# olvb/phaze

Hardware: AMD Instinct MI355X
Metric: stft_frames_per_sec_1024pt_hop256_48k (higher is better)
Workload: dtype f32+f64; 1 GPU; C2: BASELINE configs[1], mono 48 kHz 1024/256 pf 1.5, 1 ch x 2^20 hops resident; fft=1024, hop=256, channels=1, frames_per_chunk=342, parallelism=streams x1, no collective, device=AMD Radeon Graphics (gfx950:sramecc+:xna

## Files before the change

include/phaze_amd.h:

```cpp
#ifndef PHAZE_AMD_H
#define PHAZE_AMD_H

#include <stddef.h>
#include <stdint.h>

#ifdef __cplusplus
extern "C" {
#endif

#if defined(__GNUC__)
#define PV_API __attribute__((visibility("default")))
#else
#define PV_API
#endif

enum {
    PV_OK = 0,
    PV_ERR_FFT_SIZE = 1,
    PV_ERR_ARGUMENT = 2,
    PV_ERR_UNSUPPORTED = 3,
    PV_ERR_CAPACITY = 4,
    PV_ERR_DEVICE = 5,
    PV_ERR_DESTROYED = 6
};
// ... 34 lines not shown
    int32_t compute_units, device_id;
    char device_name[64];
    char kernel_name[32];
} pv_info;

PV_API int pv_create(const pv_config *cfg, pv_handle **out);
PV_API int pv_abi_version(void);
PV_API int pv_destroy(pv_handle *h);

PV_API const char *pv_last_error(const pv_handle *h);
PV_API const char *pv_status_string(int status);
PV_API int pv_get_info(const pv_handle *h, pv_info *out);
PV_API int pv_device_count(int32_t *out);

PV_API int pv_forward_stats(pv_handle *h, uint64_t *frames, uint64_t *fallbacks, int32_t reset);

PV_API int pv_reset(pv_handle *h);
PV_API int pv_reset_channels(pv_handle *h, int32_t first, int32_t count);
enum { PV_STATE_HISTORY = 1, PV_STATE_ACCUMULATOR = 2 };
PV_API int pv_reset_channels_part(pv_handle *h, int32_t first, int32_t count, int32_t parts);
PV_API int pv_get_time_cursor(const pv_handle *h, int64_t *out);
PV_API int pv_set_time_cursor(pv_handle *h, int64_t value);

PV_API int pv_export_state(pv_handle *h, int32_t ch, float *hist, float *acc, int64_t *time_cursor);
PV_API int pv_import_state(pv_handle *h, int32_t ch, const float *hist, const float *acc, int64_t time_cursor);

PV_API int pv_process(pv_handle *h, const float *const *in, float *const *out, int32_t nch,
                      int32_t nsamples, float pitch_factor);

PV_API int pv_process_begin(pv_handle *h, const float *const *in, int32_t nch, int32_t nsamples, float pitch_factor);
// ... 133 lines not shown
```

phaze_amd/capi.py:

```python
import ctypes as C
import os
import subprocess
import sys

import numpy as np

_HERE = os.path.dirname(os.path.abspath(__file__))
_LIB_PATH = os.environ.get("PHAZE_LIB") or os.path.join(_HERE, "lib", "libphaze_amd.so")
_lib = None

PV_OK, PV_ERR_FFT_SIZE, PV_ERR_ARGUMENT, PV_ERR_UNSUPPORTED, PV_ERR_CAPACITY, PV_ERR_DEVICE, PV_ERR_DESTROYED = range(7)

EXPORTS = [
    "pv_create", "pv_destroy", "pv_last_error", "pv_status_string", "pv_get_info", "pv_reset", "pv_reset_channels",
    "pv_get_time_cursor", "pv_set_time_cursor", "pv_process", "pv_process_batch", "pv_process_batch_device",
    "pv_set_stream", "pv_synchronize", "pv_debug_frame", "pv_export_state", "pv_import_state", "pv_abi_version",
    "pv_process_begin", "pv_process_end", "pv_device_count", "pv_host_alloc", "pv_host_free", "pv_reset_channels_part",
    "pv_forward_stats",
    "pv_stretch_create", "pv_stretch_destroy", "pv_stretch_reset", "pv_stretch_last_error", "pv_stretch_process", "pv_stretch_process_device",
    "pv_stretch_set_stream", "pv_stretch_synchronize", "pv_stretch_export_state", "pv_stretch_import_state",
    "pv_tempo_process", "pv_tempo_process_device",
    "pv_link_channels",
    "pv_transient_process", "pv_transient_process_device", "pv_onset_strength", "pv_onset_strength_device", "pv_transient_plan",
    "pv_onsets_from_strength", "pv_transient_chain_layout", "pv_onset_chain_layout",
    "pv_resample_create", "pv_resample_destroy", "pv_resample_reset", "pv_resample_last_error", "pv_resample_set_stream", "pv_resample_synchronize",
    "pv_resample_process", "pv_resample_process_device", "pv_resample_out_count", "pv_resample_export_state", "pv_resample_import_state",
    "pv_resample_design", "pv_resample_count",
    "pv_pitch_create", "pv_pitch_destroy", "pv_pitch_reset", "pv_pitch_last_error", "pv_pitch_set_stream", "pv_pitch_synchronize",
    "pv_pitch_process", "pv_pitch_process_device", "pv_pitch_stretch", "pv_pitch_resampler",
]


class PvError(RuntimeError):
# ... 150 lines not shown
    L.pv_pitch_stretch.argtypes = [vp]
    L.pv_pitch_resampler.argtypes = [vp]
    for n in EXPORTS:
        if n not in ("pv_last_error", "pv_status_string", "pv_stretch_last_error"):
            getattr(L, n).restype = C.c_int
    L.pv_onsets_from_strength.restype = L.pv_transient_plan.restype = C.c_int64
    L.pv_resample_design.restype = L.pv_resample_count.restype = C.c_int64
    L.pv_resample_last_error.restype = L.pv_pitch_last_error.restype = C.c_char_p
    L.pv_pitch_stretch.restype = L.pv_pitch_resampler.restype = vp
    L.pv_process_begin.argtypes = [vp, C.POINTER(fp), C.c_int32, C.c_int32, C.c_float]
    L.pv_process_end.argtypes = [vp, C.POINTER(fp)]
    L.pv_device_count.argtypes = [C.POINTER(C.c_int32)]
    L.pv_host_alloc.argtypes = [C.c_size_t, C.POINTER(vp)]
    L.pv_host_free.argtypes = [vp]
    L.pv_forward_stats.argtypes = [vp, C.POINTER(C.c_uint64), C.POINTER(C.c_uint64), C.c_int32]
    L.pv_abi_version.argtypes = []
    if L.pv_abi_version() != ABI_VERSION:
        raise PvError(PV_ERR_ARGUMENT, f"{_LIB_PATH} has PV_ABI_VERSION {L.pv_abi_version()}, this binding expects {ABI_VERSION}: rebuild the library")
    _lib = L
    return L


def _fp(a):
    return a.ctypes.data_as(C.POINTER(C.c_float))


class _PinnedBlock:

    def __init__(self, nbytes):
        self._L = load_library()
# ... 198 lines not shown
    def process_batch_device(self, d_in, d_out, nch, nhops, ch_stride, d_pitch, pitch_stride=0, channels_per_stream=1):
        self._check(self._L.pv_process_batch_device(self._h, C.c_void_p(d_in), C.c_void_p(d_out), nch, nhops, ch_stride,
                                                    C.c_void_p(d_pitch), pitch_stride, channels_per_stream))

    def set_stream(self, hip_stream):
        self._check(self._L.pv_set_stream(self._h, C.c_void_p(hip_stream)))

    def synchronize(self):
        self._check(self._L.pv_synchronize(self._h))

    def forward_stats(self, reset=False):
        a, b = C.c_uint64(0), C.c_uint64(0)
        self._check(self._L.pv_forward_stats(self._h, C.byref(a), C.byref(b), 1 if reset else 0))
        return int(a.value), int(b.value)

    def debug_frame(self, ch, block, pitch):
        N = self.fft_size
        H = N // 2 + 1
        block = np.ascontiguousarray(block, dtype=np.float32)
        X = np.zeros(2 * N, dtype=np.float64)
        mag = np.zeros(H, dtype=np.float32)
        flags = np.zeros(H, dtype=np.int32)
        Y = np.zeros(2 * H, dtype=np.float32)
        self._check(self._L.pv_debug_frame(self._h, ch, _fp(block), C.c_float(float(pitch)), X.ctypes.data_as(C.POINTER(C.c_double)),
                                           _fp(mag), flags.ctypes.data_as(C.POINTER(C.c_int32)), _fp(Y)))
        return {"X": X, "mag": mag, "flags": flags, "Y": Y}


def tempo_hops(tempo, synthesis_hop, min_hop, max_hop, carry=0.0):
    t = np.atleast_1d(np.asarray(tempo, np.float64))
# ... 467 lines not shown
```

phaze_amd/csrc/pv_capi.hip:

```cpp
#include <hip/hip_runtime.h>
#include <math.h>
#include <stdio.h>
#include <stdlib.h>
#include <string.h>

#include <atomic>
#include <chrono>
#include <vector>
#if defined(__x86_64__)
#include <immintrin.h>
#endif

#include "../../include/phaze_amd.h"
#include "pv_kernels.h"

namespace {
constexpr uint32_t kMagic = 0x50564d49u;
constexpr int kHdrFloats = 16;
constexpr int kMaxPieces = 16;
constexpr int kFwdStatWords = 1024;
thread_local char g_create_err[256] = "";
}

struct pv_handle {
    uint32_t magic;
    int N, hop, L, R, log2n;
    int max_channels, max_hops, device, cus;
    int frames_per_chunk_cfg;
    int last_frames_per_chunk;
    hipStream_t own_stream, stream;
    double2 *d_tw64;
    float2 *d_tw32;
    float *d_hann;
    float *d_hist[2], *d_acc[2];
    int cur;
    float *d_stage_in, *d_stage_out, *d_pitch;
    unsigned *d_chain_list;
    long chain_list_cap;
    int chain_list_flip = 0;
    unsigned char *d_gscratch;
    size_t gscratch_cap;
    float *d_snap;
    size_t snap_floats;
    unsigned idle_ticks;
// ... 52 lines not shown
int fail_hip(pv_handle *h, hipError_t e, const char *what)
{
    char buf[256];
    snprintf(buf, sizeof buf, "%s: %s", what, hipGetErrorString(e));
    return fail(h, PV_ERR_DEVICE, buf);
}

#define HIPCHK(h, call)                                            \
    do {                                                           \
        hipError_t e_ = (call);                                    \
        if (e_ != hipSuccess) return fail_hip((h), e_, #call);     \
    } while (0)

bool live(const pv_handle *h) { return h && h->magic == kMagic; }

int pick_frames_per_chunk(const pv_handle *h, int nch, int nhops)
{
    if (h->frames_per_chunk_cfg > 0) return h->frames_per_chunk_cfg;
    long per_cu;
    if (h->use_wave2k) per_cu = pv_wave2k_threads() / 64;
    else if (h->use_wave) per_cu = pv_wave_threads() / 64;
    else if (h->use_wg) { per_cu = (160 * 1024) / (long)(pv_wg_lds_bytes(h->log2n, h->hop, !h->use_wg16) + 256); if (per_cu < 1) per_cu = 1; }
    else { per_cu = (160 * 1024) / (long)pv_kernel_lds_bytes(h->log2n, h->hop); if (per_cu > 8) per_cu = 8; if (per_cu < 1) per_cu = 1; }
    const long resident = per_cu * h->cus;
    const int R = h->R;
    int best = R > 1 ? R : 1;
    double best_eff = -1.0;
    auto consider = [&](int F) {
        if (F < 1) return;
        const long chunks = (nhops + F - 1) / F;
        const long chains = (long)nch * chunks;
        const long rounds = (chains + resident - 1) / resident;
        const double fill = (double)chains / (double)(rounds * resident);
        const double halo = (double)nhops / (double)(nhops + (chunks - 1) * (R - 1));
        const double eff = fill * halo;
        if (eff > best_eff + 1e-9) { best_eff = eff; best = F; }
// ... 6 lines not shown
    for (int F = 48 * R; F >= (R > 1 ? R : 1); F -= (F > 8 * R ? R : 1)) {
        if (F > nhops && F > R) continue;
        consider(F);
    }
    if (best > nhops) best = nhops;
    return best < 1 ? 1 : best;
}

int launch_chain(pv_handle *h, const float *d_in, float *d_out, int ch0, int nch, int nhops, long ch_stride, const float *d_pitch,
                 int pitch_stride, int ch_per_stream, bool chunked, int dbg_ch, unsigned done_seq, int spread = -1)
{
    PvKernelParams p;
    memset(&p, 0, sizeof p);
    p.in = d_in; p.out = d_out; p.ch_stride = ch_stride;
    p.nhops = nhops; p.hop = h->hop;
    p.frames_per_chunk = chunked ? pick_frames_per_chunk(h, nch, nhops) : nhops;
    p.pitch = d_pitch; p.pitch_stride = pitch_stride; p.ch_per_stream = ch_per_stream > 0 ? ch_per_stream : 1;
    const size_t soff = (size_t)ch0 * h->L;
    p.hist_in = h->d_hist[h->cur] + soff; p.hist_out = h->d_hist[h->cur ^ 1] + soff;
    p.acc_in = h->d_acc[h->cur] + soff;   p.acc_out = h->d_acc[h->cur ^ 1] + soff;
    p.t0_mod_n = (int)(h->time_cursor & (int64_t)(h->N - 1));
    p.tw64 = h->d_tw64; p.tw32 = h->d_tw32; p.hann = h->d_hann;
    p.dbg_ch = -1; p.dbg_frame = -1;
    p.fwd64 = h->fwd64 ? 1 : 0; p.fwd_stats = h->d_fwd_stats;
    if (done_seq) { p.done = h->d_done; p.done_seq = done_seq; }
#ifdef PV_STAMPS
    p.stamps = h->d_stamps;
#endif
    if (dbg_ch >= 0) { p.dbg_X = h->d_dbgX; p.dbg_mag = h->d_dbgMag; p.dbg_flags = h->d_dbgFlags; p.dbg_Y = h->d_dbgY; p.dbg_ch = dbg_ch; p.dbg_frame = 0; }
    const int nchunks = (nhops + p.frames_per_chunk - 1) / p.frames_per_chunk;
    h->last_frames_per_chunk = p.frames_per_chunk;
// ... 22 lines not shown
        if (!h->use_wave && !h->use_wg) {
            const size_t stride = pv_kernel_gscratch_bytes(h->log2n, h->hop);
            if (stride) {
                const size_t need = stride * (size_t)nch * (size_t)nchunks;
                if (need > ((size_t)16 << 30)) return fail(h, PV_ERR_CAPACITY, "fft_size >= 16384: the launch needs more than 16 GiB of scratch (fewer channels or hops per call)");
                if (need > h->gscratch_cap) {
                    HIPCHK(h, hipStreamSynchronize(h->stream));
                    if (h->d_gscratch) (void)hipFree(h->d_gscratch);
                    h->d_gscratch = nullptr; h->gscratch_cap = 0;
                    HIPCHK(h, hipMalloc(&h->d_gscratch, need));
                    h->gscratch_cap = need;
                }
                p.gscratch = h->d_gscratch; p.gscratch_stride = stride;
            }
        }
        e = h->use_wave ? pv_launch_wave(p, nch, nchunks, h->stream, spread, list, list_next)
          : h->use_wg ? pv_launch_wg(h->log2n, p, nch, nchunks, h->stream, !h->use_wg16)
                      : pv_launch_chain(h->log2n, p, nch, nchunks, h->stream);
    }
    if (e != hipSuccess) return fail_hip(h, e, "kernel launch");
    return PV_OK;
}

int commit_chain(pv_handle *h, int nch, int nhops)
{
    if (nch > h->used_channels) h->used_channels = nch;
    if (nch < h->used_channels && h->L > 0) {
        const size_t off = (size_t)nch * h->L, cnt = (size_t)(h->used_channels - nch) * h->L * sizeof(float);
        HIPCHK(h, hipMemcpyAsync(h->d_hist[h->cur ^ 1] + off, h->d_hist[h->cur] + off, cnt, hipMemcpyDeviceToDevice, h->stream));
        HIPCHK(h, hipMemcpyAsync(h->d_acc[h->cur ^ 1] + off, h->d_acc[h->cur] + off, cnt, hipMemcpyDeviceToDevice, h->stream));
    }
    h->cur ^= 1;
    h->time_cursor += (int64_t)nhops * h->hop;
// ... 445 lines not shown
int pv_forward_stats(pv_handle *h, uint64_t *frames, uint64_t *fallbacks, int32_t reset)
{
    if (!live(h)) return PV_ERR_DESTROYED;
    { const int rs_ = resident_stop(h); if (rs_ != PV_OK) return rs_; }
    HIPCHK(h, hipSetDevice(h->device));
    HIPCHK(h, hipStreamSynchronize(h->stream));
    unsigned long long st[256];
    HIPCHK(h, hipMemcpy(st, h->d_fwd_stats, sizeof st, hipMemcpyDeviceToHost));
    uint64_t a = 0, b = 0;
    for (int i = 0; i < 128; i++) { a += st[2 * i]; b += st[2 * i + 1]; }
    if (frames) *frames = a;
    if (fallbacks) *fallbacks = b;
    if (reset) HIPCHK(h, hipMemset(h->d_fwd_stats, 0, sizeof(unsigned long long) * kFwdStatWords));
    return PV_OK;
}

#ifdef PV_FLIP_COUNT
PV_API int pv_exp_flip_stats(pv_handle *h, uint64_t *out)
{
    if (!live(h) || !out) return PV_ERR_ARGUMENT;
    HIPCHK(h, hipSetDevice(h->device));
    HIPCHK(h, hipStreamSynchronize(h->stream));
    unsigned long long st[kFwdStatWords];
    HIPCHK(h, hipMemcpy(st, h->d_fwd_stats, sizeof st, hipMemcpyDeviceToHost));
    for (int k = 0; k < 12; k++) out[k] = 0;
    for (int i = 0; i < 128; i++) { out[0] += st[2 * i]; out[1] += st[2 * i + 1]; out[2] += st[256 + 2 * i]; out[3] += st[257 + 2 * i]; }
    for (int k = 0; k < 6; k++) out[4 + k] = st[512 + k] & 0xFFFFFFFFull;
    out[10] = st[600]; out[11] = st[601];
    return PV_OK;
}
// ... 333 lines not shown
```

phaze_amd/csrc/pv_kernels.h:

```cpp
#pragma once
#include <hip/hip_runtime.h>
#include <stddef.h>
#include <atomic>

struct PvKernelParams {
    const float *in;
    float *out;
    long ch_stride;
    int nhops;
    int hop;
    int frames_per_chunk;
    int nchunks;
    int nch;
    const float *pitch;
    int pitch_stride;
    int ch_per_stream;
    const float *hist_in;
    float *hist_out;
    const float *acc_in;
    float *acc_out;
    int t0_mod_n;
    const double2 *tw64;
    const float2 *tw32;
    const float *hann;
// ... 40 lines not shown
inline PvKernelParams pv_resident_params(const PvKernelParams &p, int nslots)
{
    PvKernelParams q = p;
    q.nchunks = 1; q.nch = nslots; q.nhops = 1; q.frames_per_chunk = 1;
    return q;
}

int pv_kernel_threads(int log2n);
size_t pv_kernel_lds_bytes(int log2n, int hop);
size_t pv_kernel_gscratch_bytes(int log2n, int hop);
hipError_t pv_launch_chain(int log2n, const PvKernelParams &p, int nch, int nchunks, hipStream_t st);

size_t pv_wave_lds_bytes();
int pv_wave_threads();
bool pv_wave_supported(int log2n, int hop);
hipError_t pv_launch_wave(const PvKernelParams &p, int nch, int nchunks, hipStream_t st, int spread, unsigned *list, unsigned *list_next = nullptr);
hipError_t pv_launch_wave_resident(const PvKernelParams &p, int nslots, hipStream_t st);
hipError_t pv_launch_wave2k_resident(const PvKernelParams &p, int nslots, hipStream_t st);
bool pv_wg_resident_supported(int log2n, int hop, bool wg8);
hipError_t pv_launch_wg_resident(int log2n, const PvKernelParams &p, int nslots, hipStream_t st, bool wg8);

bool pv_wave2k_supported(int log2n, int hop);
size_t pv_wave2k_lds_bytes();
int pv_wave2k_threads();
hipError_t pv_launch_wave2k(const PvKernelParams &p, int nch, int nchunks, hipStream_t st);

bool pv_wg_supported(int log2n, int hop);
size_t pv_wg_lds_bytes(int log2n, int hop, bool wg8);
int pv_wg_threads(int log2n, int hop, bool wg8);
hipError_t pv_launch_wg(int log2n, const PvKernelParams &p, int nch, int nchunks, hipStream_t st, bool wg8);

bool pv_wg16_supported(int log2n, int hop);
// ... 6 lines not shown
```

phaze_amd/csrc/pv_wave_kernel.hip:

```cpp
#include <hip/hip_runtime.h>
#include <stdint.h>
#include <type_traits>

#include "pv_kernels.h"
#include "pv_device_common.h"
#include "pv_pk_math.h"
#include "pv_residue.h"
#include "pv_wave_fft.h"
#include "pv_guard.h"

namespace {

#ifndef PV_FP64_FLAVOUR
#define PV_FP64_FLAVOUR 0
#endif
#ifndef PV_WAVES
#define PV_WAVES (PV_FP64_FLAVOUR ? 8 : 12)
#endif
#ifndef PV_WAVES_PER_SIMD
#define PV_WAVES_PER_SIMD (PV_FP64_FLAVOUR ? 2 : 3)
#endif
constexpr bool FP64 = PV_FP64_FLAVOUR != 0;
constexpr int WAVES = PV_WAVES;
constexpr int RES_WAVES = 4;
// ... 1245 lines not shown
    __syncthreads();
    if (threadIdx.x == 0) {
        unsigned n[2] = {0u, 0u};
        for (int w = 0; w < CLS_WAVES; w++) if (cls_of[w] < 2u) n[cls_of[w]]++;
        base[0] = n[0] ? atomicAdd(&list[0], n[0]) : 0u;
        base[1] = n[1] ? atomicAdd(&list[1], n[1]) : 0u;
    }
    __syncthreads();
    if (l == 0 && cls < 2u) {
        unsigned before = 0;
        for (int w = 0; w < wv; w++) before += (cls_of[w] == cls) ? 1u : 0u;
        list[2 + cls * nchains + base[cls] + before] = (unsigned)chain;
    }
}

template <int S_ROWS, bool AUX>
hipError_t launch_wave(const PvKernelParams &p, int nch, int nchunks, hipStream_t st, int spread, unsigned *list, unsigned *list_next)
{
    constexpr bool F32OK = !AUX && !FP64;
    const bool f32 = F32OK && !p.fwd64;
    PvKernelParams q = p;
    q.nchunks = nchunks;
    q.nch = nch;
    const long chains = (long)nch * nchunks;
    const dim3 grid((unsigned)((chains + WAVES - 1) / WAVES), 1, 1), block(64 * WAVES, 1, 1);
    const size_t lds = pv_wave_lds_bytes();
    auto k = [&] { return f32 ? pv_launch_instance<pv_wave_kernel_1024<S_ROWS, AUX, false, false, F32OK>>(grid, block, lds, st, q)
                              : pv_launch_instance<pv_wave_kernel_1024<S_ROWS, AUX, false, false, false>>(grid, block, lds, st, q); };
    auto ks = [&] { return f32 ? pv_launch_instance<pv_wave_kernel_1024<S_ROWS, false, false, true, F32OK>>(grid, block, lds, st, q)
                               : pv_launch_instance<pv_wave_kernel_1024<S_ROWS, false, false, true>>(grid, block, lds, st, q); };
    if (FP64 && !AUX) return ks();
    if (AUX || spread == 0 || (spread < 0 && !list)) return k();
    if (spread > 0) return ks();
    if (!list_next) {
        hipError_t e = hipMemsetAsync(list, 0, 2 * sizeof(unsigned), st);
        if (e != hipSuccess) return e;
    }
    hipLaunchKernelGGL(pv_classify_chains<S_ROWS>, dim3((unsigned)((chains + CLS_WAVES - 1) / CLS_WAVES), 1, 1), dim3(64 * CLS_WAVES, 1, 1), 0, st, q, list, list_next);
    q.chain_count = list;
    q.chain_list = list + 2;
    const hipError_t e = ks();
    return e != hipSuccess ? e : k();
}

template <int S_ROWS>
hipError_t launch_wave_resident(const PvKernelParams &p, int nslots, hipStream_t st)
{
    const dim3 grid((unsigned)((nslots + RES_WAVES - 1) / RES_WAVES), 1, 1), block(64 * RES_WAVES, 1, 1);
    const PvKernelParams q = pv_resident_params(p, nslots);
    return (!FP64 && !p.fwd64) ? pv_launch_instance<pv_wave_kernel_1024<S_ROWS, false, true, false, !FP64>>(grid, block, pv_wave_lds_bytes(), st, q)
                               : pv_launch_instance<pv_wave_kernel_1024<S_ROWS, false, true, false, false>>(grid, block, pv_wave_lds_bytes(), st, q);
}

}

size_t pv_wave_lds_bytes() { return TAB_BYTES + WAVES * WAVE_LDS; }

int pv_wave_threads() { return 64 * WAVES; }

bool pv_wave_supported(int log2n, int hop) { return log2n == 10 && (hop == 128 || hop == 256 || hop == 512 || hop == 1024); }

hipError_t pv_launch_wave_resident(const PvKernelParams &p, int nslots, hipStream_t st)
{
    switch (p.hop) {
    case 128: return launch_wave_resident<1>(p, nslots, st);
    case 256: return launch_wave_resident<2>(p, nslots, st);
    case 512: return launch_wave_resident<4>(p, nslots, st);
    case 1024: return launch_wave_resident<8>(p, nslots, st);
    default: return hipErrorInvalidValue;
    }
}

hipError_t pv_launch_wave(const PvKernelParams &p, int nch, int nchunks, hipStream_t st, int spread, unsigned *list, unsigned *list_next)
// ... 11 lines not shown
```

Baseline: 615.4 million frames/s.

## Add 16-wave-per-workgroup kernel for classified hop-256 spread chains

Adds a new wave4 kernel that packs 16 waves per workgroup with a smaller per-wave LDS carve for the classified 'spread' chain list at hop 256 in f32. It is dispatched in place of the old spread kernel. The chunk-size heuristic now sizes chunks for 16 chains per CU when classification is active. The aim is higher occupancy and better CU fill for the spread path. In exchange it adds a large duplicate kernel plus a launch counter API, and risks register pressure under the 4-block launch bound.

```diff
diff --git a/include/phaze_amd.h b/include/phaze_amd.h
--- a/include/phaze_amd.h
+++ b/include/phaze_amd.h
@@ -72,6 +72,7 @@
 PV_API int pv_device_count(int32_t *out);
 
 PV_API int pv_forward_stats(pv_handle *h, uint64_t *frames, uint64_t *fallbacks, int32_t reset);
+PV_API int64_t pv_wave4_launches(pv_handle *h);
 
 PV_API int pv_reset(pv_handle *h);
 PV_API int pv_reset_channels(pv_handle *h, int32_t first, int32_t count);
diff --git a/phaze_amd/capi.py b/phaze_amd/capi.py
--- a/phaze_amd/capi.py
+++ b/phaze_amd/capi.py
@@ -16,7 +16,7 @@
     "pv_get_time_cursor", "pv_set_time_cursor", "pv_process", "pv_process_batch", "pv_process_batch_device",
     "pv_set_stream", "pv_synchronize", "pv_debug_frame", "pv_export_state", "pv_import_state", "pv_abi_version",
     "pv_process_begin", "pv_process_end", "pv_device_count", "pv_host_alloc", "pv_host_free", "pv_reset_channels_part",
-    "pv_forward_stats",
+    "pv_forward_stats", "pv_wave4_launches",
     "pv_stretch_create", "pv_stretch_destroy", "pv_stretch_reset", "pv_stretch_last_error", "pv_stretch_process", "pv_stretch_process_device",
     "pv_stretch_set_stream", "pv_stretch_synchronize", "pv_stretch_export_state", "pv_stretch_import_state",
     "pv_tempo_process", "pv_tempo_process_device",
@@ -197,6 +197,9 @@
     L.pv_host_alloc.argtypes = [C.c_size_t, C.POINTER(vp)]
     L.pv_host_free.argtypes = [vp]
     L.pv_forward_stats.argtypes = [vp, C.POINTER(C.c_uint64), C.POINTER(C.c_uint64), C.c_int32]
+    if hasattr(L, "pv_wave4_launches"):
+        L.pv_wave4_launches.argtypes = [vp]
+        L.pv_wave4_launches.restype = C.c_int64
     L.pv_abi_version.argtypes = []
     if L.pv_abi_version() != ABI_VERSION:
         raise PvError(PV_ERR_ARGUMENT, f"{_LIB_PATH} has PV_ABI_VERSION {L.pv_abi_version()}, this binding expects {ABI_VERSION}: rebuild the library")
@@ -425,6 +428,9 @@
         self._check(self._L.pv_forward_stats(self._h, C.byref(a), C.byref(b), 1 if reset else 0))
         return int(a.value), int(b.value)
 
+    def wave4_launches(self):
+        return int(self._L.pv_wave4_launches(self._h))
+
     def debug_frame(self, ch, block, pitch):
         N = self.fft_size
         H = N // 2 + 1
diff --git a/phaze_amd/csrc/pv_capi.hip b/phaze_amd/csrc/pv_capi.hip
--- a/phaze_amd/csrc/pv_capi.hip
+++ b/phaze_amd/csrc/pv_capi.hip
@@ -28,6 +28,7 @@
     int max_channels, max_hops, device, cus;
     int frames_per_chunk_cfg;
     int last_frames_per_chunk;
+    long long wave4_launches;
     hipStream_t own_stream, stream;
     double2 *d_tw64;
     float2 *d_tw32;
@@ -110,12 +111,12 @@
 
 bool live(const pv_handle *h) { return h && h->magic == kMagic; }
 
-int pick_frames_per_chunk(const pv_handle *h, int nch, int nhops)
+int pick_frames_per_chunk(const pv_handle *h, int nch, int nhops, bool classified = false)
 {
     if (h->frames_per_chunk_cfg > 0) return h->frames_per_chunk_cfg;
     long per_cu;
     if (h->use_wave2k) per_cu = pv_wave2k_threads() / 64;
-    else if (h->use_wave) per_cu = pv_wave_threads() / 64;
+    else if (h->use_wave) per_cu = classified ? pv_wave_batch_chains_per_cu(h->hop, h->fwd64) : pv_wave_threads() / 64;
     else if (h->use_wg) { per_cu = (160 * 1024) / (long)(pv_wg_lds_bytes(h->log2n, h->hop, !h->use_wg16) + 256); if (per_cu < 1) per_cu = 1; }
     else { per_cu = (160 * 1024) / (long)pv_kernel_lds_bytes(h->log2n, h->hop); if (per_cu > 8) per_cu = 8; if (per_cu < 1) per_cu = 1; }
     const long resident = per_cu * h->cus;
@@ -152,7 +153,7 @@
     memset(&p, 0, sizeof p);
     p.in = d_in; p.out = d_out; p.ch_stride = ch_stride;
     p.nhops = nhops; p.hop = h->hop;
-    p.frames_per_chunk = chunked ? pick_frames_per_chunk(h, nch, nhops) : nhops;
+    p.frames_per_chunk = chunked ? pick_frames_per_chunk(h, nch, nhops, h->use_wave && spread < 0 && dbg_ch < 0) : nhops;
     p.pitch = d_pitch; p.pitch_stride = pitch_stride; p.ch_per_stream = ch_per_stream > 0 ? ch_per_stream : 1;
     const size_t soff = (size_t)ch0 * h->L;
     p.hist_in = h->d_hist[h->cur] + soff; p.hist_out = h->d_hist[h->cur ^ 1] + soff;
@@ -205,9 +206,11 @@
                 p.gscratch = h->d_gscratch; p.gscratch_stride = stride;
             }
         }
+        const unsigned long long w4_before = pv_wave4_launches_this_thread();
         e = h->use_wave ? pv_launch_wave(p, nch, nchunks, h->stream, spread, list, list_next)
           : h->use_wg ? pv_launch_wg(h->log2n, p, nch, nchunks, h->stream, !h->use_wg16)
                       : pv_launch_chain(h->log2n, p, nch, nchunks, h->stream);
+        h->wave4_launches += (long long)(pv_wave4_launches_this_thread() - w4_before);
     }
     if (e != hipSuccess) return fail_hip(h, e, "kernel launch");
     return PV_OK;
@@ -683,6 +686,8 @@
     if (reset) HIPCHK(h, hipMemset(h->d_fwd_stats, 0, sizeof(unsigned long long) * kFwdStatWords));
     return PV_OK;
 }
+
+int64_t pv_wave4_launches(pv_handle *h) { return live(h) ? (int64_t)h->wave4_launches : -1; }
 
 #ifdef PV_FLIP_COUNT
 PV_API int pv_exp_flip_stats(pv_handle *h, uint64_t *out)
diff --git a/phaze_amd/csrc/pv_kernels.h b/phaze_amd/csrc/pv_kernels.h
--- a/phaze_amd/csrc/pv_kernels.h
+++ b/phaze_amd/csrc/pv_kernels.h
@@ -78,8 +78,14 @@
 size_t pv_wave_lds_bytes();
 int pv_wave_threads();
 bool pv_wave_supported(int log2n, int hop);
+int pv_wave_batch_chains_per_cu(int hop, bool fwd64);
 hipError_t pv_launch_wave(const PvKernelParams &p, int nch, int nchunks, hipStream_t st, int spread, unsigned *list, unsigned *list_next = nullptr);
 hipError_t pv_launch_wave_resident(const PvKernelParams &p, int nslots, hipStream_t st);
+
+bool pv_wave4_covers(int log2n, int hop);
+int pv_wave4_chains_per_workgroup();
+hipError_t pv_launch_wave4(const PvKernelParams &p, long chains, hipStream_t st);
+unsigned long long pv_wave4_launches_this_thread();
 hipError_t pv_launch_wave2k_resident(const PvKernelParams &p, int nslots, hipStream_t st);
 bool pv_wg_resident_supported(int log2n, int hop, bool wg8);
 hipError_t pv_launch_wg_resident(int log2n, const PvKernelParams &p, int nslots, hipStream_t st, bool wg8);
diff --git a/phaze_amd/csrc/pv_wave4_kernel.hip b/phaze_amd/csrc/pv_wave4_kernel.hip
--- /dev/null
+++ b/phaze_amd/csrc/pv_wave4_kernel.hip
@@ -0,0 +1,553 @@
+#include <hip/hip_runtime.h>
+#include <stdint.h>
+#include <type_traits>
+
+#include "pv_kernels.h"
+#include "pv_device_common.h"
+#include "pv_pk_math.h"
+#include "pv_wave_fft.h"
+#include "pv_guard.h"
+
+namespace {
+
+constexpr int W4_WAVES = 16;
+constexpr int T4_TW1F = 0;
+constexpr int T4_TW2F = T4_TW1F + 4 * 64 * 16;
+constexpr int T4_HANN = T4_TW2F + 4 * 8 * 16;
+constexpr int T4_BYTES = T4_HANN + 4 * 64 * 16;
+constexpr int O4_Y = 0;
+constexpr int O4_XV = 0;
+constexpr int O4_MAG = 4112;
+constexpr int O4_ROUTE = 4352;
+constexpr int O4_PSH = O4_ROUTE + 528 * 4;
+constexpr int W4_LDS = 9216;
+static_assert(O4_PSH + 1024 <= W4_LDS, "per-wave carve");
+static_assert(O4_MAG + 520 * 4 <= O4_PSH && O4_MAG >= 257 * 16, "magnitudes sit behind the fp64 partner rows and in front of the shift table");
+static_assert(T4_BYTES + W4_WAVES * W4_LDS <= 163840, "tables + 16 x the per-wave carve must fit the 160 KB of a CU");
+
+__device__ __forceinline__ int opaque(int v) { asm volatile("" : "+v"(v)); return v; }
+
+__device__ __attribute__((noinline)) void w4_build_shift_table(float f, unsigned wave_off, int l)
+{
+    constexpr int N = 1024, H = 513, DROP = 0x4000;
+    extern __shared__ __attribute__((aligned(16))) unsigned char smem_all[];
+    short *DSH = reinterpret_cast<short *>(smem_all + wave_off + O4_PSH);
+    const double pf = (double)f;
+#pragma unroll
+    for (int r = 0; r < 8; r++) {
+        const int pk = l + 64 * r;
+        const double ps = floor((double)pk * pf + 0.5);
+        const bool ok = (ps <= (double)H) && (ps >= -(double)(2 * N));
+        DSH[pk] = ok ? (short)((int)ps - pk) : (short)DROP;
+    }
+}
+
+__device__ __forceinline__ void w4_spectrum32(const float2 (&raw)[8], unsigned char *smem, int l, pk::c32 wlfs, float isc_)
+{
+    extern __shared__ __attribute__((aligned(16))) unsigned char smem_all[];
+    const v4f *TW1F4 = reinterpret_cast<const v4f *>(smem_all + T4_TW1F);
+    const v4f *TW2F4 = reinterpret_cast<const v4f *>(smem_all + T4_TW2F);
+    const v4f *HW4 = reinterpret_cast<const v4f *>(smem_all + T4_HANN);
+    float *MAG = reinterpret_cast<float *>(smem + O4_MAG);
+    float2 *XV = reinterpret_cast<float2 *>(smem + O4_XV);
+    pv_prio(PH_FA);
+    pk::c32 zc[8];
+#pragma unroll
+    for (int j = 0; j < 4; j++) {
+        const v4f h = HW4[j * 64 + l];
+        zc[2 * j] = pk::mul_conj(pk::c32{raw[2 * j].x, raw[2 * j].y}, pk::c32{h.x, h.y});
+        zc[2 * j + 1] = pk::mul_conj(pk::c32{raw[2 * j + 1].x, raw[2 * j + 1].y}, pk::c32{h.z, h.w});
+    }
+    fft512_wave_inv_pk<true, NoStamp, true>(zc, reinterpret_cast<pk::c32 *>(smem), TW1F4, TW2F4, l);
+    pv_prio(PH_SPLITX);
+    pk::c32 *XCH = reinterpret_cast<pk::c32 *>(smem);
+#pragma unroll
+    for (int r = 4; r < 8; r++) XCH[(r - 4) * 64 + l] = zc[r];
+    if (l == 0) XCH[256] = zc[0];
+    wave_sync();
+    pv_prio(PH_SPLITM);
+    const pk::c32 isc{isc_, isc_};
+    pk::c32 zm[4];
+#pragma unroll
+    for (int r = 0; r < 4; r++) zm[r] = XCH[(3 - r) * 64 + 64 - l];
+    wave_sync();
+#pragma unroll
+    for (int r = 0; r < 4; r++) {
+        const pk::c32 E = pk::add_conj(zc[r], zm[r]), O = pk::sub_conj(zc[r], zm[r]);
+        const pk::c32 T = pk::cmul(mul_w16_inv_pk(O, r), wlfs);
+        const pk::c32 xa = pk::conj_fma_j(T, isc, E), xb = pk::fnma_j(T, isc, E);
+        MAG[4 + l + 64 * r] = mag32(xa);
+        MAG[4 + 512 - l - 64 * r] = mag32(xb);
+        XV[r * 64 + l] = float2{xa.x, xa.y};
+        XV[(4 + r) * 64 + l] = float2{xb.x, xb.y};
+    }
+    if (l == 0) { const pk::c32 x256{2.0f * zc[4].x, 2.0f * zc[4].y}; MAG[4 + 256] = mag32(x256); XV[512] = float2{x256.x, x256.y}; }
+}
+
+__device__ __forceinline__ void w4_fft512_f64(double2 (&a)[8], double2 *S, const double2 *__restrict__ tw64, int l)
+{
+    const int lh = l >> 3, ll = l & 7;
+    radix8<double, false>(a);
+#pragma unroll
+    for (int k = 1; k < 8; k++) a[k] = cmul(a[k], tw64[(2 * l * k) & 1023]);
+    {
+        unsigned w[8][4];
+#pragma unroll
+        for (int k = 0; k < 8; k++) {
+            const uint2 x = __builtin_bit_cast(uint2, a[k].x), y = __builtin_bit_cast(uint2, a[k].y);
+            w[k][0] = x.x; w[k][1] = x.y; w[k][2] = y.x; w[k][3] = y.y;
+        }
+        transpose_hi3_regs<4>(w);
+#pragma unroll
+        for (int k = 0; k < 8; k++) {
+            a[k].x = __builtin_bit_cast(double, uint2{w[k][0], w[k][1]});
+            a[k].y = __builtin_bit_cast(double, uint2{w[k][2], w[k][3]});
+        }
+    }
+    radix8<double, false>(a);
+#pragma unroll
+    for (int k = 1; k < 8; k++) a[k] = cmul(a[k], tw64[(16 * ll * k) & 1023]);
+    pv_prio(PH_FX);
+#pragma unroll
+    for (int k = 0; k < 8; k++) S[k * TP + lh * 8 + ((ll + lh) & 7)] = a[k];
+    wave_sync();
+#pragma unroll
+    for (int n = 0; n < 8; n++) a[n] = S[lh * TP + ll * 8 + ((n + ll) & 7)];
+    wave_sync();
+    pv_prio(PH_FP3);
+    radix8<double, false>(a);
+}
+
+template <int S_ROWS>
+__device__ __attribute__((noinline)) PV_NO_DS_MERGE void w4_forward_cold(const float *in, const float *hist, int hist_len, bool vec_in, int frame, int wide,
+                                                                        const double2 *__restrict__ tw64, pk::c32 wlfs, float isc, unsigned wave_off, int l)
+{
+    constexpr int N = 1024, HOP = 128 * S_ROWS;
+    extern __shared__ __attribute__((aligned(16))) unsigned char smem_all[];
+    unsigned char *smem = smem_all + wave_off;
+    const WaveSrc src{in, hist, hist_len, false};
+    float2 raw[8];
+    {
+        const long s0 = (long)(frame + 1) * HOP - N + 2 * l;
+#pragma unroll
+        for (int r = 0; r < 8; r++) {
+            const long sx = s0 + 128 * r;
+            if (vec_in) raw[r] = *reinterpret_cast<const float2 *>(sx < 0 ? src.hist + sx + src.hist_len : src.in + sx);
+            else raw[r] = float2{src.at(sx), src.at(sx + 1)};
+        }
+    }
+    if (!wide) { w4_spectrum32(raw, smem, l, wlfs, isc); return; }
+    const v4f *HW4 = reinterpret_cast<const v4f *>(smem_all + T4_HANN);
+    float *MAG = reinterpret_cast<float *>(smem + O4_MAG);
+    float2 *XV = reinterpret_cast<float2 *>(smem + O4_XV);
+    double2 *S64 = reinterpret_cast<double2 *>(smem);
+    const v4u psh = *reinterpret_cast<const v4u *>(smem + O4_PSH + 16 * l);
+    const double2 wl = tw64[l];
+    pv_prio(PH_FA);
+    double2 z[8];
+#pragma unroll
+    for (int j = 0; j < 4; j++) {
+        const v4f h = HW4[j * 64 + l];
+        const v2f xw0 = v2f{raw[2 * j].x, raw[2 * j].y} * pk::c32{h.x, h.y}, xw1 = v2f{raw[2 * j + 1].x, raw[2 * j + 1].y} * pk::c32{h.z, h.w};
+        z[2 * j] = double2{(double)xw0.x, (double)xw0.y};
+        z[2 * j + 1] = double2{(double)xw1.x, (double)xw1.y};
+    }
+    w4_fft512_f64(z, S64, tw64, l);
+    pv_prio(PH_SPLITX);
+#pragma unroll
+    for (int r = 4; r < 8; r++) S64[(r - 4) * 64 + l] = z[r];
+    wave_sync();
+    pv_prio(PH_SPLITM);
+    float2 XA[4], XB[4], x256f{0.f, 0.f};
+#pragma unroll
+    for (int r = 0; r < 4; r++) {
+        const double2 zm = S64[(3 - r) * 64 + 64 - l];
+        const double2 E{z[r].x + zm.x, z[r].y - zm.y};
+        const double2 O{z[r].x - zm.x, z[r].y + zm.y};
+        const double2 WO = cmul(wl, mul_w16<double, false>(O, r));
+        double2 xa{E.x + WO.y, E.y - WO.x};
+        double2 xb{E.x - WO.y, -(E.y + WO.x)};
+        if (r == 0 && l == 0) {
+            xa = double2{2.0 * (z[0].x + z[0].y), 0.0};
+            xb = double2{2.0 * (z[0].x - z[0].y), 0.0};
+        }
+        MAG[4 + l + 64 * r] = (float)(xa.x * xa.x + xa.y * xa.y);
+        MAG[4 + 512 - l - 64 * r] = (float)(xb.x * xb.x + xb.y * xb.y);
+        XA[r] = float2{(float)xa.x, (float)xa.y};
+        XB[r] = float2{(float)xb.x, (float)xb.y};
+    }
+    if (l == 0) {
+        const double2 x256{2.0 * z[4].x, -2.0 * z[4].y};
+        MAG[4 + 256] = (float)(x256.x * x256.x + x256.y * x256.y);
+        x256f = float2{(float)x256.x, (float)x256.y};
+    }
+    wave_sync();
+#pragma unroll
+    for (int r = 0; r < 4; r++) { XV[r * 64 + l] = XA[r]; XV[(4 + r) * 64 + l] = XB[r]; }
+    if (l == 0) XV[512] = x256f;
+    *reinterpret_cast<v4u *>(smem + O4_PSH + 16 * l) = psh;
+}
+
+template <int S_ROWS>
+__global__ __launch_bounds__(64 * W4_WAVES, 4) PV_NO_DS_MERGE void pv_wave4_kernel_1024(const PvKernelParams p)
+{
+    constexpr int N = 1024, H = 513;
+    constexpr int HOP = 128 * S_ROWS, R = N / HOP, LROWS = 8 - S_ROWS;
+    const int l = threadIdx.x & 63;
+    const int wv = __builtin_amdgcn_readfirstlane(threadIdx.x >> 6);
+    if ((long)blockIdx.x >= (long)p.chain_count[0]) return;
+    long chain = (long)wv * gridDim.x + blockIdx.x;
+    const long total = (long)p.nch * p.nchunks;
+    const bool listed = chain < (long)p.chain_count[0];
+    chain = listed ? (long)p.chain_list[chain] : total;
+    const int ch = (int)(chain / p.nchunks), chunk = (int)(chain - (long)ch * p.nchunks);
+
+    extern __shared__ __attribute__((aligned(16))) unsigned char smem_all[];
+    const v4f *TW1F4 = reinterpret_cast<const v4f *>(smem_all + T4_TW1F);
+    const v4f *TW2F4 = reinterpret_cast<const v4f *>(smem_all + T4_TW2F);
+    const v4f *HW4 = reinterpret_cast<const v4f *>(smem_all + T4_HANN);
+    {
+        float2 *t1f = reinterpret_cast<float2 *>(smem_all + T4_TW1F);
+        float2 *t2f = reinterpret_cast<float2 *>(smem_all + T4_TW2F);
+        float2 *hh = reinterpret_cast<float2 *>(smem_all + T4_HANN);
+        if (threadIdx.x < 512) {
+            const int i = threadIdx.x, k = i >> 6, ln = i & 63;
+            const double2 w = p.tw64[(2 * ln * k) & (N - 1)];
+            t1f[2 * ((k >> 1) * 64 + ln) + (k & 1)] = float2{(float)w.x, -(float)w.y};
+            hh[2 * ((k >> 1) * 64 + ln) + (k & 1)] = float2{0.5f * p.hann[2 * i], 0.5f * p.hann[2 * i + 1]};
+            if (i < 64) {
+                const int k2 = i >> 3, n0 = i & 7;
+                const double2 w2 = p.tw64[(16 * n0 * k2) & (N - 1)];
+                t2f[2 * ((k2 >> 1) * 8 + n0) + (k2 & 1)] = float2{(float)w2.x, -(float)w2.y};
+            }
+        }
+    }
+    __syncthreads();
+    if (!listed || ch >= p.nch) return;
+
+    const unsigned wave_off = T4_BYTES + wv * W4_LDS;
+    unsigned char *smem = smem_all + wave_off;
+    unsigned psh_key = 0u;
+    bool psh_valid = false;
+    unsigned pred = 0;
+
+    const int first_out = chunk * p.frames_per_chunk;
+    int last_out = first_out + p.frames_per_chunk;
+    if (last_out > p.nhops) last_out = p.nhops;
+    int first_frame = first_out - (R - 1);
+    const bool from_state = (first_frame <= 0);
+    if (from_state) first_frame = 0;
+
+    const long cbase = (long)ch * p.ch_stride;
+    const WaveSrc src{p.in + cbase, p.hist_in + (long)ch * (N - HOP), N - HOP, false};
+    float *outp = p.out + cbase;
+    const bool vec_out = (reinterpret_cast<uintptr_t>(outp) & 7u) == 0;
+    const bool vec_in = ((reinterpret_cast<uintptr_t>(src.in) | reinterpret_cast<uintptr_t>(src.hist)) & 7u) == 0;
+    const float *pitch_row = p.pitch + (p.pitch_stride ? (long)(ch / p.ch_per_stream) * p.pitch_stride : 0);
+
+    const float2 wlf = cconj(p.tw32[l]);
+    constexpr float SC = 2.0f / ((float)N * (float)R);
+    const pk::c32 wlfs{wlf.x * SC, wlf.y * SC};
+
+    float2 acc[8];
+#pragma unroll
+    for (int r = 0; r < 8; r++) acc[r] = float2{0.f, 0.f};
+    if (from_state) {
+#pragma unroll
+        for (int r = 0; r < LROWS; r++) {
+            const float *a = p.acc_in + (long)ch * (N - HOP) + 2 * l + 128 * r;
+            acc[r] = float2{a[0], a[1]};
+        }
+    }
+    float2 raw[8];
+    auto load_window = [&](int frame, int lq) {
+        const long s0 = (long)(frame + 1) * HOP - N + 2 * lq;
+#pragma unroll
+        for (int r = 0; r < 8; r++) {
+            const long sx = s0 + 128 * r;
+            if (vec_in) raw[r] = *reinterpret_cast<const float2 *>(sx < 0 ? src.hist + sx + src.hist_len : src.in + sx);
+            else raw[r] = float2{src.at(sx), src.at(sx + 1)};
+        }
+    };
+    load_window(first_frame, l);
+    float pf_next = pitch_row[first_frame];
+    int emit_v = first_out;
+    asm volatile("" : "+v"(emit_v));
+    unsigned n_fallback = 0;
+
+    for (int m = first_frame; m < last_out; ++m) {
+        const float pfm = __uint_as_float(__builtin_amdgcn_readfirstlane(__float_as_uint(pf_next)));
+        const int tmod = (int)(((long)p.t0_mod_n + (long)m * HOP) & (N - 1));
+        int lq = opaque(l);
+        float *MAG = reinterpret_cast<float *>(smem + O4_MAG);
+        const short *DSH = reinterpret_cast<const short *>(smem + O4_PSH);
+        {
+            const unsigned pfb = __float_as_uint(pfm);
+            if (!psh_valid || pfb != psh_key) { psh_key = pfb; psh_valid = true; w4_build_shift_table(pfm, wave_off, l); }
+        }
+        auto cold = [&](int wide) {
+            w4_forward_cold<S_ROWS>(src.in, src.hist, src.hist_len, vec_in, m, wide, p.tw64, wlfs, 1.0f / SC, wave_off, l);
+        };
+        const bool wide_first = pred >= PRED_WIDE;
+        if (wide_first) cold(1); else w4_spectrum32(raw, smem, lq, wlfs, 1.0f / SC);
+        wave_sync();
+        pv_prio(PH_PEAKS);
+        int last_peak = -1, last_shift = 0;
+        bool nonfinite = false;
+        unsigned rt[8];
+        unsigned rt512 = NOROUTE;
+        {
+            unsigned mg[12];
+            unsigned pm[11], nm[8];
+            v4u dq;
+            typedef const volatile __attribute__((address_space(3))) v2u *lds_v2u;
+            typedef const volatile __attribute__((address_space(3))) v4u *lds_v4u;
+            auto read_mags = [&]() {
+                const v2u q0 = *(lds_v2u)(&MAG[4 + 8 * lq - 2]);
+                const v4u q1 = *(lds_v4u)(&MAG[4 + 8 * lq]);
+                const v4u q2 = *(lds_v4u)(&MAG[4 + 8 * lq + 4]);
+                const v2u q3 = *(lds_v2u)(&MAG[4 + 8 * lq + 8]);
+                dq = *(lds_v4u)(&DSH[8 * lq]);
+                mg[0] = q0.x; mg[1] = q0.y; mg[2] = q1.x; mg[3] = q1.y; mg[4] = q1.z; mg[5] = q1.w;
+                mg[6] = q2.x; mg[7] = q2.y; mg[8] = q2.z; mg[9] = q2.w; mg[10] = q3.x; mg[11] = q3.y;
+#pragma unroll
+                for (int j = 3; j < 11; j++) pm[j] = max(mg[j], mg[j + 1]);
+#pragma unroll
+                for (int i = 0; i < 8; i++) nm[i] = max(max(mg[i], mg[i + 1]), pm[i + 3]);
+            };
+            bool fl[8];
+            auto take_flags = [&]() {
+#pragma unroll
+                for (int i = 0; i < 8; i++) {
+                    const bool in_range = (i < 2) ? (l != 0) : (i == 7) ? (l != 63) : true;
+                    fl[i] = in_range & (nm[i] < mg[i + 2]);
+                }
+            };
+            auto in_band = [&](float K, float Rr) -> bool {
+                const pk::c32 KK{K, K}, RR{Rr, Rr};
+                float tmin = 1.0f;
+#pragma unroll
+                for (int j = 0; j < 4; j++) {
+                    const int i = 2 * j;
+                    const pk::c32 c2{__uint_as_float(mg[i + 2]), __uint_as_float(mg[i + 3])}, n2{__uint_as_float(nm[i]), __uint_as_float(nm[i + 1])};
+                    const pk::c32 d2 = pk::sub(c2, n2), s2 = pk::add(c2, n2);
+                    pk::c32 t2 = pk::fms(d2, d2, pk::mul(pk::fma(s2, RR, KK), s2));
+                    if (j == 0 && l == 0) t2 = pk::c32{1.f, 1.f};
+                    if (j == 3 && l == 63) t2.y = 1.f;
+                    tmin = fminf(fminf(tmin, t2.x), t2.y);
+                }
+                return !(K > 0.f) | (tmin <= 0.f);
+            };
+            auto frame_max = [&]() { return wave_max_u32(max(max(max(pm[3], pm[5]), max(pm[7], pm[9])), mg[2])); };
+            read_mags();
+            take_flags();
+            bool fall = true;
+            if (!wide_first) fall = __any(in_band(guard_k_of(frame_max()), GUARD_R));
+            if (fall) {
+                auto recold = [&](int wide) {
+                    cold(wide);
+                    wave_sync();
+                    pv_prio(PH_PEAKS);
+                    lq = opaque(l);
+                    read_mags();
+                    take_flags();
+                };
+                if (!wide_first) recold(1);
+                const unsigned mb = frame_max();
+                const bool out_sure = mb < GUARD_M_MIN_BITS - GUARD_M_SLACK || mb >= GUARD_M_MAX_BITS + GUARD_M_SLACK;
+                const bool in_sure = mb >= GUARD_M_MIN_BITS + GUARD_M_SLACK && mb < GUARD_M_MAX_BITS - GUARD_M_SLACK;
+                const bool sure_b = out_sure || (in_sure && __any(in_band(GUARD_CKN * __uint_as_float(mb), GUARD_RN)));
+                bool class_b = true;
+                if (wide_first && !sure_b) {
+                    recold(0);
+                    class_b = __any(in_band(guard_k_of(frame_max()), GUARD_R));
+                    if (class_b) recold(1);
+                }
+                pred = (class_b && sure_b) ? min(pred + 1u, (unsigned)PRED_MAX) : (pred > 3u ? pred - 3u : 0u);
+                n_fallback += class_b ? 1u : 0u;
+            } else {
+                pred = pred > 3u ? pred - 3u : 0u;
+            }
+            {
+                const int mn = (m + 1 < last_out) ? m + 1 : m;
+                load_window(mn, lq);
+                pf_next = pitch_row[mn];
+            }
+            nonfinite = __any(max(max(max(pm[3], pm[5]), max(pm[7], pm[9])), mg[2]) >= 0x7F800000u);
+            constexpr int NEGPD = -(2048 << 16), POSPD = 4096 << 16;
+            int pd[8];
+#pragma unroll
+            for (int i = 0; i < 8; i++)
+                pd[i] = (int)__builtin_amdgcn_perm((unsigned)(8 * lq + i), dq[i >> 1], (i & 1) ? 0x05040302u : 0x05040100u);
+            int lastown[8], firstown[8];
+            int cur = NEGPD;
+#pragma unroll
+            for (int i = 0; i < 8; i++) { cur = fl[i] ? pd[i] : cur; lastown[i] = cur; }
+            int nx = POSPD;
+#pragma unroll
+            for (int i = 7; i >= 0; i--) { firstown[i] = nx; nx = fl[i] ? pd[i] : nx; }
+            const int last_in = cur, first_in = nx;
+            const unsigned long long occ = __ballot(cur >= 0);
+            const unsigned long long below = occ & ((1ull << l) - 1ull);
+            const unsigned long long above = (l == 63) ? 0ull : (occ >> (l + 1));
+            const int src_lo = below ? 63 - __clzll((long long)below) : 0;
+            const int src_hi = above ? l + __ffsll((long long)above) : 0;
+            int cprev = __shfl(last_in, src_lo, 64), cnext = __shfl(first_in, src_hi, 64);
+            if (!below) cprev = NEGPD;
+            if (!above) cnext = POSPD;
+            if (occ == 0ull) {
+#pragma unroll
+                for (int i = 0; i < 8; i++) rt[i] = NOROUTE;
+            } else {
+                const int lp = __shfl(last_in, 63 - __clzll((long long)occ), 64);
+                last_peak = lp >> 16;
+                last_shift = (int)(short)(lp & 0xFFFF);
+                auto route_of = [&](int b, int pp, int pn) -> unsigned {
+                    const int own = (b - (pp >> 16) < (pn >> 16) - b) ? pp : pn;
+                    const int delta = __builtin_amdgcn_sbfe(own, 0, 16);
+                    return __builtin_amdgcn_perm((unsigned)__mul24(delta, tmod), (unsigned)(b + delta), 0x05040100u);
+                };
+#pragma unroll
+                for (int i = 0; i < 8; i++) rt[i] = route_of(8 * lq + i, max(lastown[i], cprev), min(firstown[i], cnext));
+                if (l == 63) rt512 = route_of(512, max(last_in, cprev), POSPD);
+            }
+        }
+        (void)last_peak; (void)last_shift;
+        pv_prio(PH_SCATTER);
+        pk::c32 zi[8];
+        {
+            lq = opaque(l);
+            wave_sync();
+            float2 *Yn = reinterpret_cast<float2 *>(smem + O4_Y);
+            const float2 *XV = reinterpret_cast<const float2 *>(smem + O4_XV);
+            unsigned *ROUTE = reinterpret_cast<unsigned *>(smem + O4_ROUTE);
+            *reinterpret_cast<uint4 *>(&ROUTE[8 * lq]) = uint4{rt[0], rt[1], rt[2], rt[3]};
+            *reinterpret_cast<uint4 *>(&ROUTE[8 * lq + 4]) = uint4{rt[4], rt[5], rt[6], rt[7]};
+            if (l == 63) ROUTE[512] = rt512;
+            float2 XA[4], XB[4];
+#pragma unroll
+            for (int r = 0; r < 4; r++) { XA[r] = XV[r * 64 + lq]; XB[r] = XV[(4 + r) * 64 + lq]; }
+            const float2 x256f = XV[512];
+            wave_sync();
+#pragma unroll
+            for (int r = 0; r < 4; r++) *reinterpret_cast<v4f *>(&Yn[2 * lq + 128 * r]) = v4f{0.f, 0.f, 0.f, 0.f};
+            if (l == 0) Yn[512] = float2{0.f, 0.f};
+            wave_sync();
+            auto rot_mode = [&](auto mode_tag, unsigned r_, float2 v) -> float2 {
+                constexpr int MODE = decltype(mode_tag)::value;
+                if (MODE == 0) return v;
+                if (MODE == 2) {
+                    const unsigned sg = (r_ << 6) & 0x80000000u;
+                    return float2{__uint_as_float(__float_as_uint(v.x) ^ sg), __uint_as_float(__float_as_uint(v.y) ^ sg)};
+                }
+                return rotate_route<R, 10>(r_, v, p.tw32);
+            };
+            auto scatter = [&](auto mode_tag) {
+#pragma unroll
+                for (int r = 0; r < 4; r++) {
+                    const unsigned ra = ROUTE[lq + 64 * r], ta = ra & 0xFFFFu;
+                    const unsigned rb = ROUTE[512 - lq - 64 * r], tb = rb & 0xFFFFu;
+                    if (ta < (unsigned)H) Yn[ta] = rot_mode(mode_tag, ra, XA[r]);
+                    if (tb < (unsigned)H) Yn[tb] = rot_mode(mode_tag, rb, XB[r]);
+                }
+                if (l == 0) { const unsigned r256 = ROUTE[256], tg = r256 & 0xFFFFu; if (tg < (unsigned)H) Yn[tg] = rot_mode(mode_tag, r256, x256f); }
+            };
+            if (tmod == 0) scatter(std::integral_constant<int, 0>{});
+            else if (tmod == N / 2) scatter(std::integral_constant<int, 2>{});
+            else scatter(std::integral_constant<int, 1>{});
+            if (nonfinite && l == 0) Yn[1] = float2{__uint_as_float(0x7FC00000u), __uint_as_float(0x7FC00000u)};
+            wave_sync();
+            pv_prio(PH_C2R);
+            lq = opaque(l);
+            const unsigned char *Yb = smem + O4_Y;
+            const unsigned ystr = 8u * (unsigned)lq, ystr_m = 8u * (unsigned)(512 - 192 - lq);
+            const float sc = SC;
+            const pk::c32 scsc{sc, sc};
+            pk::c32 zb[4];
+#pragma unroll
+            for (int r = 0; r < 4; r++) {
+                pk::c32 yk = *reinterpret_cast<const pk::c32 *>(Yb + ystr + 512 * r), ym = *reinterpret_cast<const pk::c32 *>(Yb + ystr_m + 512 * (3 - r));
+                if (r == 0 && l == 0) { yk.y = 0.f; ym.y = 0.f; }
+                const pk::c32 E = pk::add_conj(yk, ym), O = pk::sub_conj(yk, ym);
+                const pk::c32 c = pk::cmul(mul_w16_inv_pk(O, r), wlfs);
+                zi[r] = pk::fma_addj(E, scsc, c);
+                zb[r] = pk::fma_conj_subj(E, scsc, c);
+            }
+            const pk::c32 y256 = *reinterpret_cast<const pk::c32 *>(Yb + 2048);
+            pk::c32 *XCH = reinterpret_cast<pk::c32 *>(smem + O4_ROUTE);
+#pragma unroll
+            for (int r = 0; r < 4; r++) XCH[r * 64 + lq] = zb[r];
+            wave_sync();
+#pragma unroll
+            for (int r = 0; r < 4; r++) zi[7 - r] = XCH[r * 64 + 64 - lq];
+            if (l == 0) zi[4] = pk::c32{2.0f * y256.x * sc, -2.0f * y256.y * sc};
+            wave_sync();
+            fft512_wave_inv_pk(zi, reinterpret_cast<pk::c32 *>(smem), TW1F4, TW2F4, opaque(l));
+        }
+#pragma unroll
+        for (int r = 0; r < 8; r++) asm volatile("" :: "v"(raw[r]));
+        asm volatile("" :: "v"(pf_next));
+        pv_prio(PH_OLA);
+        {
+            const bool emit_out = (m >= emit_v);
+            lq = opaque(l);
+            float2 fr[8];
+#pragma unroll
+            for (int j = 0; j < 4; j++) {
+                const v4f h = HW4[j * 64 + lq];
+                const pk::c32 f0 = pk::mul(zi[2 * j], pk::c32{h.x, h.y}), f1 = pk::mul(zi[2 * j + 1], pk::c32{h.z, h.w});
+                fr[2 * j] = float2{f0.x, f0.y};
+                fr[2 * j + 1] = float2{f1.x, f1.y};
+            }
+#pragma unroll
+            for (int r = 0; r < S_ROWS; r++) {
+                const float2 o{acc[r].x + fr[r].x, acc[r].y + fr[r].y};
+                if (emit_out) {
+                    float *dst = outp + (long)m * HOP + 2 * l + 128 * r;
+                    if (vec_out) __builtin_nontemporal_store(v2f{o.x, o.y}, reinterpret_cast<v2f *>(dst));
+                    else { __builtin_nontemporal_store(o.x, dst); __builtin_nontemporal_store(o.y, dst + 1); }
+                }
+            }
+#pragma unroll
+            for (int r = 0; r < LROWS; r++) {
+                const int s = r + S_ROWS;
+                acc[r] = (s < LROWS) ? float2{acc[s].x + fr[s].x, acc[s].y + fr[s].y} : fr[s];
+            }
+        }
+    }
+
+    if (p.fwd_stats && l == 0) {
+        unsigned long long *st = p.fwd_stats + 2 * (chain & 127);
+        atomicAdd(st, (unsigned long long)(last_out - first_frame));
+        if (n_fallback) atomicAdd(st + 1, (unsigned long long)n_fallback);
+    }
+    if (chunk == p.nchunks - 1) {
+#pragma unroll
+        for (int r = 0; r < LROWS; r++) {
+            float *a = p.acc_out + (long)ch * (N - HOP) + 2 * l + 128 * r;
+            a[0] = acc[r].x; a[1] = acc[r].y;
+            float *hs = p.hist_out + (long)ch * (N - HOP) + 2 * l + 128 * r;
+            hs[0] = raw[r + S_ROWS].x; hs[1] = raw[r + S_ROWS].y;
+        }
+    }
+    pv_signal_done<false>(p.done, p.done_seq, chain);
+}
+
+thread_local unsigned long long w4_launches = 0;
+
+}
+
+bool pv_wave4_covers(int log2n, int hop) { return log2n == 10 && hop == 256; }
+
+int pv_wave4_chains_per_workgroup() { return W4_WAVES; }
+
+unsigned long long pv_wave4_launches_this_thread() { return w4_launches; }
+
+hipError_t pv_launch_wave4(const PvKernelParams &q, long chains, hipStream_t st)
+{
+    if (!q.chain_list || !q.chain_count || q.fwd64 || q.hop != 256) return hipErrorInvalidValue;
+    const dim3 grid((unsigned)((chains + W4_WAVES - 1) / W4_WAVES), 1, 1), block(64 * W4_WAVES, 1, 1);
+    const hipError_t e = pv_launch_instance<pv_wave4_kernel_1024<2>>(grid, block, (size_t)(T4_BYTES + W4_WAVES * W4_LDS), st, q);
+    if (e == hipSuccess) w4_launches++;
+    return e;
+}
diff --git a/phaze_amd/csrc/pv_wave_kernel.hip b/phaze_amd/csrc/pv_wave_kernel.hip
--- a/phaze_amd/csrc/pv_wave_kernel.hip
+++ b/phaze_amd/csrc/pv_wave_kernel.hip
@@ -1283,6 +1283,16 @@
     }
 }
 
+inline bool wave4_dispatch(int hop, bool fwd64)
+{
+#if PV_FP64_FLAVOUR || defined(PV_FLIP_COUNT)
+    (void)hop; (void)fwd64;
+    return false;
+#else
+    return !fwd64 && pv_wave4_covers(10, hop);
+#endif
+}
+
 template <int S_ROWS, bool AUX>
 hipError_t launch_wave(const PvKernelParams &p, int nch, int nchunks, hipStream_t st, int spread, unsigned *list, unsigned *list_next)
 {
@@ -1308,7 +1318,7 @@
     hipLaunchKernelGGL(pv_classify_chains<S_ROWS>, dim3((unsigned)((chains + CLS_WAVES - 1) / CLS_WAVES), 1, 1), dim3(64 * CLS_WAVES, 1, 1), 0, st, q, list, list_next);
     q.chain_count = list;
     q.chain_list = list + 2;
-    const hipError_t e = ks();
+    const hipError_t e = (f32 && wave4_dispatch(p.hop, p.fwd64 != 0)) ? pv_launch_wave4(q, chains, st) : ks();
     return e != hipSuccess ? e : k();
 }
 
@@ -1326,6 +1336,8 @@
 size_t pv_wave_lds_bytes() { return TAB_BYTES + WAVES * WAVE_LDS; }
 
 int pv_wave_threads() { return 64 * WAVES; }
+
+int pv_wave_batch_chains_per_cu(int hop, bool fwd64) { return wave4_dispatch(hop, fwd64) ? pv_wave4_chains_per_workgroup() : WAVES; }
 
 bool pv_wave_supported(int log2n, int hop) { return log2n == 10 && (hop == 128 || hop == 256 || hop == 512 || hop == 1024); }
 
```

After: 540.1 million frames/s. -12.2%, worse.
